# enoche/MMRec

Hardware: NVIDIA H100
Metric: graph-prop edges/sec (+ full-catalog scored-items/sec in extra) @ d=64 (higher is better)
Workload: dtype f32

## Files before the change

include/mmrec_b200.h:

```cpp
#ifndef MMREC_B200_H
#define MMREC_B200_H

#include <stddef.h>
#include <stdint.h>

#ifdef __cplusplus
extern "C" {
#endif

#define MMREC_OK 0
#define MMREC_EINVAL (-1)
#define MMREC_EWORKSPACE (-2)
#define MMREC_ECUDA (-3)
#define MMREC_EUNSUPPORTED (-4)

#define MMREC_ABI_VERSION 3

int mmrec_abi_version(void);
const char* mmrec_last_error(void);
int mmrec_device_check(void);
int64_t mmrec_launch_count(void);

size_t mmrec_csr_from_coo_workspace_bytes(int64_t nnz, int64_t n_rows);
int mmrec_csr_from_coo(int64_t nnz, const int64_t* row, const int64_t* col, const float* val,
// ... 16 lines not shown
                   const int32_t* rowptr, const int32_t* colidx, const float* vals,
                   const int32_t* tasks, int64_t n_tasks, int64_t n_cta_tasks, const int32_t* split_rows,
                   int32_t* counters, float* partial,
                   const float* X, int64_t ldx,
                   float* Y, int64_t ldy,
                   const float* acc_in, float* acc_out, int64_t ldacc, float acc_div,
                   const float* gate_ref, int64_t ldgate,
                   void* stream);

int mmrec_spmm_acc_f32(int64_t n_rows, int64_t n_cols, int d,
                       const int32_t* rowptr, const int32_t* colidx, const float* vals,
                       const int32_t* tasks, int64_t n_tasks, int64_t n_cta_tasks, const int32_t* split_rows,
                       int32_t* counters, float* partial,
                       const float* X, int64_t ldx, float* Y, int64_t ldy,
                       const float* acc_in, float* acc_out, int64_t ldacc, float acc_div, int y_accumulate, void* stream);

int mmrec_spmm_drop_f32(int64_t n_rows, int64_t n_cols, int d,
                        const int32_t* rowptr, const int32_t* colidx, const float* vals,
                        const int32_t* tasks, int64_t n_tasks, int64_t n_cta_tasks, const int32_t* split_rows,
                        int32_t* counters, float* partial,
                        const float* X, int64_t ldx, float* Y, int64_t ldy,
                        const float* acc_in, float* acc_out, int64_t ldacc, float acc_div,
                        const uint32_t* keep_bits, float scale, void* stream);

int mmrec_edge_keep_bits(int64_t nnz, const float* draws, float keep_prob, const int32_t* draw_of, const int32_t* mirror,
                         uint32_t* keep_bits, uint32_t* keep_bits_t, void* stream);

typedef struct {
    int64_t n_rows, n_cols;
    const int32_t* rowptr; const int32_t* colidx; const float* vals;
    const int32_t* tasks; int64_t n_tasks, n_cta_tasks; const int32_t* split_rows; int32_t* counters; float* partial;
    const float* X; int64_t ldx;
    float* Y; int64_t ldy;
    const float* acc_in; float* acc_out; int64_t ldacc; float acc_div;
    const float* post; int64_t ldpost; int64_t post_row0;
    int sync_before;
} mmrec_spmm_step;
int mmrec_spmm_chain_f32(int d, int n_steps, const mmrec_spmm_step* steps, void* stream);

typedef struct {
    mmrec_spmm_step step;
    const float* X_hi; int64_t ldx_hi; int64_t x_split;
    const float* acc_in_hi; int64_t ldacc_in_hi; int64_t acc_in_split;
} mmrec_spmm_step2;
int mmrec_spmm_steps_f32(int d, int n_steps, const mmrec_spmm_step2* steps, int cooperative, void* stream);

int mmrec_project_set_path(int tensor_core);
size_t mmrec_project_workspace_bytes(int64_t n_out, int64_t F, int d);
int mmrec_project_f32(int64_t n_out, const int64_t* idx, const float* table, int64_t n_table, int64_t F,
                      const float* W, const float* bias, int d, int l2_normalize,
                      float* Y, int64_t ldy, void* ws, size_t ws_bytes, void* stream);

int mmrec_debug_mma_rate(int kind, int N, int iters, int distinct, long long* cycles_per_cta, void* stream);

int mmrec_debug_stream_probe(const float* table, int64_t n_rows, int64_t F, int R, int burst_bytes, int ctas_per_sm, float* sink,
                             void* stream);

int mmrec_score_set_path(int path);
size_t mmrec_score_workspace_bytes(int64_t B, int64_t n_items, int d);
int mmrec_score_f32(int64_t B, const int64_t* users, const float* Ue, int64_t ldu,
                    int64_t n_items, const float* Ie, int64_t ldi, int d,
                    float* S, int64_t ldS, void* ws, size_t ws_bytes, void* stream);
int mmrec_mask_f32(int64_t mask_nnz, const int64_t* mask_rows, const int64_t* mask_cols,
                   int64_t B, int64_t n_items, int64_t item_offset, float* S, int64_t ldS, void* stream);
int mmrec_topk_rows_f32(int64_t B, int64_t n_items, const float* S, int64_t ldS, int k,
                        int64_t item_offset, int64_t* out_idx, float* out_val, void* stream);
size_t mmrec_score_topk_workspace_bytes(int64_t B, int64_t n_items, int d, int k);
int mmrec_score_topk_f32(int64_t B, const int64_t* users, const float* Ue, int64_t ldu,
                         int64_t n_items, const float* Ie, int64_t ldi, int d,
                         int64_t mask_nnz, const int64_t* mask_rows, const int64_t* mask_cols,
                         int k, int64_t item_offset, int64_t* out_idx, float* out_val,
                         void* ws, size_t ws_bytes, void* stream);
size_t mmrec_catalog_bytes(int64_t n_items, int d);
int mmrec_catalog_pack_f32(int64_t n_items, const float* Ie, int64_t ldi, int d,
                           void* cat, size_t cat_bytes, void* stream);
int mmrec_score_topk_cat_f32(int64_t B, const int64_t* users, const float* Ue, int64_t ldu,
                             int64_t n_items, const float* Ie, int64_t ldi, int d, const void* cat,
                             int64_t mask_nnz, const int64_t* mask_rows, const int64_t* mask_cols,
                             int k, int64_t item_offset, int64_t* out_idx, float* out_val,
                             void* ws, size_t ws_bytes, void* stream);
int64_t mmrec_debug_fused_fallback_rows(const void* ws, int64_t B, int64_t n_items, int d, int k, int64_t mask_nnz, int with_cat);
int mmrec_debug_cf_scratch(int64_t B, int64_t n_items, int d, int k, int64_t mask_nnz, int with_cat, int64_t* out, int cap);
int mmrec_debug_cf_timing(float* us, int cap);

size_t mmrec_knn_topk_workspace_bytes(int64_t n, int F, int64_t m, int k);
int mmrec_knn_topk_f32(int64_t n, const float* X, int64_t ldx, int F, int64_t m, const int64_t* rows, int k,
                       int64_t* out_idx, float* out_val, void* ws, size_t ws_bytes, void* stream);
int64_t mmrec_debug_knn_fallback_rows(void);
int mmrec_debug_knn_scratch(int64_t n, int F, int64_t m, int k, int64_t* out, int cap);
int mmrec_knn_topk_shrink_f32(int64_t n, const float* X, int64_t ldx, int F, int64_t m, const int64_t* rows, int k,
                              const float* norms, float shrink, int64_t* out_idx, float* out_val, void* ws, size_t ws_bytes,
                              void* stream);

int mmrec_sparse_scores_f32(int64_t B, const int64_t* users, int64_t n_items, const int32_t* r_ptr, const int32_t* r_col,
                            const float* r_val, const int32_t* s_ptr, const int32_t* s_col, const float* s_val, float* out,
                            int64_t ldo, void* stream);
size_t mmrec_sparse_score_topk_workspace_bytes(int64_t B, int64_t n_items, int64_t mask_nnz, int k);
int mmrec_sparse_score_topk_f32(int64_t B, const int64_t* users, int64_t n_items, const int32_t* r_ptr, const int32_t* r_col,
                                const float* r_val, const int32_t* s_ptr, const int32_t* s_col, const float* s_val,
                                int64_t mask_nnz, const int64_t* mask_rows, const int64_t* mask_cols, int k,
                                int64_t* out_idx, float* out_val, void* ws, size_t ws_bytes, void* stream);
int64_t mmrec_debug_sparse_topk_fallback_rows(void);

size_t mmrec_expsum_rows_workspace_bytes(int64_t B, int64_t M, int d);
int mmrec_expsum_rows_f32(int64_t B, const float* Q, int64_t ldq, int64_t M, const float* T, int64_t ldt, int d, float inv_tau,
                          float* ttl, void* ws, size_t ws_bytes, void* stream);
// ... 50 lines not shown
```

mmrec_b200/_lib.py:

```python
from __future__ import annotations

import ctypes as C
import os

_HERE = os.path.dirname(os.path.abspath(__file__))
LIB_PATH = os.path.join(_HERE, "csrc", "libmmrec_b200.so")

_i64, _i32, _f32, _f64, _sz, _p = C.c_int64, C.c_int, C.c_float, C.c_double, C.c_size_t, C.c_void_p

PROTOTYPES = {
    "mmrec_abi_version": (_i32, []),
    "mmrec_last_error": (C.c_char_p, []),
    "mmrec_device_check": (_i32, []),
    "mmrec_launch_count": (_i64, []),
    "mmrec_csr_from_coo_workspace_bytes": (_sz, [_i64, _i64]),
    "mmrec_csr_from_coo": (_i32, [_i64, _p, _p, _p, _i64, _i64, _i32, _p, _p, _p, _p, _p, _sz, _p]),
    "mmrec_spmm_plan_workspace_bytes": (_sz, [_i64, _i64]),
    "mmrec_spmm_plan": (_i32, [_i64, _p, _i32, _i32, _i64, _p, _p, _p, _p, _sz, _p]),
    "mmrec_bipartite_norm_workspace_bytes": (_sz, [_i64, _i64]),
    "mmrec_bipartite_norm_f32": (_i32, [_i64, _p, _p, _i64, _i64, _f32, _p, _p, _sz, _p]),
    "mmrec_spmm_set_lanes": (_i32, [_i32]),
    "mmrec_spmm_f32": (_i32, [_i64, _i64, _i32, _p, _p, _p, _p, _i64, _i64, _p, _p, _p, _p, _i64, _p, _i64, _p, _p, _i64,
                              _f32, _p, _i64, _p]),
    "mmrec_spmm_acc_f32": (_i32, [_i64, _i64, _i32, _p, _p, _p, _p, _i64, _i64, _p, _p, _p, _p, _i64, _p, _i64, _p, _p, _i64,
                                  _f32, _i32, _p]),
    "mmrec_spmm_drop_f32": (_i32, [_i64, _i64, _i32, _p, _p, _p, _p, _i64, _i64, _p, _p, _p, _p, _i64, _p, _i64, _p, _p, _i64,
                                   _f32, _p, _f32, _p]),
    "mmrec_edge_keep_bits": (_i32, [_i64, _p, _f32, _p, _p, _p, _p, _p]),
    "mmrec_spmm_chain_f32": (_i32, [_i32, _i32, _p, _p]),
    "mmrec_spmm_steps_f32": (_i32, [_i32, _i32, _p, _i32, _p]),
    "mmrec_project_set_path": (_i32, [_i32]),
    "mmrec_project_workspace_bytes": (_sz, [_i64, _i64, _i32]),
    "mmrec_project_f32": (_i32, [_i64, _p, _p, _i64, _i64, _p, _p, _i32, _i32, _p, _i64, _p, _sz, _p]),
    "mmrec_debug_mma_rate": (_i32, [_i32, _i32, _i32, _i32, _p, _p]),
    "mmrec_debug_stream_probe": (_i32, [_p, _i64, _i64, _i32, _i32, _i32, _p, _p]),
    "mmrec_score_set_path": (_i32, [_i32]),
    "mmrec_score_workspace_bytes": (_sz, [_i64, _i64, _i32]),
    "mmrec_score_f32": (_i32, [_i64, _p, _p, _i64, _i64, _p, _i64, _i32, _p, _i64, _p, _sz, _p]),
    "mmrec_mask_f32": (_i32, [_i64, _p, _p, _i64, _i64, _i64, _p, _i64, _p]),
    "mmrec_topk_rows_f32": (_i32, [_i64, _i64, _p, _i64, _i32, _i64, _p, _p, _p]),
    "mmrec_score_topk_workspace_bytes": (_sz, [_i64, _i64, _i32, _i32]),
    "mmrec_score_topk_f32": (_i32, [_i64, _p, _p, _i64, _i64, _p, _i64, _i32, _i64, _p, _p, _i32, _i64, _p, _p, _p,
                                    _sz, _p]),
    "mmrec_catalog_bytes": (_sz, [_i64, _i32]),
    "mmrec_catalog_pack_f32": (_i32, [_i64, _p, _i64, _i32, _p, _sz, _p]),
    "mmrec_score_topk_cat_f32": (_i32, [_i64, _p, _p, _i64, _i64, _p, _i64, _i32, _p, _i64, _p, _p, _i32, _i64, _p, _p, _p,
                                        _sz, _p]),
    "mmrec_debug_cf_timing": (_i32, [_p, _i32]),
    "mmrec_debug_fused_fallback_rows": (_i64, [_p, _i64, _i64, _i32, _i32, _i64, _i32]),
    "mmrec_debug_cf_scratch": (_i32, [_i64, _i64, _i32, _i32, _i64, _i32, _p, _i32]),
    "mmrec_knn_topk_workspace_bytes": (_sz, [_i64, _i32, _i64, _i32]),
    "mmrec_knn_topk_f32": (_i32, [_i64, _p, _i64, _i32, _i64, _p, _i32, _p, _p, _p, _sz, _p]),
    "mmrec_debug_knn_fallback_rows": (_i64, []),
    "mmrec_debug_knn_scratch": (_i32, [_i64, _i32, _i64, _i32, _p, _i32]),
    "mmrec_knn_topk_shrink_f32": (_i32, [_i64, _p, _i64, _i32, _i64, _p, _i32, _p, _f32, _p, _p, _p, _sz, _p]),
    "mmrec_sparse_scores_f32": (_i32, [_i64, _p, _i64, _p, _p, _p, _p, _p, _p, _p, _i64, _p]),
    "mmrec_sparse_score_topk_workspace_bytes": (_sz, [_i64, _i64, _i64, _i32]),
    "mmrec_sparse_score_topk_f32": (_i32, [_i64, _p, _i64, _p, _p, _p, _p, _p, _p, _i64, _p, _p, _i32, _p, _p, _p, _sz, _p]),
    "mmrec_debug_sparse_topk_fallback_rows": (_i64, []),
    "mmrec_expsum_rows_workspace_bytes": (_sz, [_i64, _i64, _i32]),
    "mmrec_expsum_rows_f32": (_i32, [_i64, _p, _i64, _i64, _p, _i64, _i32, _f32, _p, _p, _sz, _p]),
    "mmrec_expsum_rows_bwd_f32": (_i32, [_i64, _p, _i64, _i64, _p, _i64, _i32, _f32, _p, _p, _i64, _p, _i64, _p, _sz, _p]),
    "mmrec_topk_merge": (_i32, [_i32, _i64, _i32, _p, _p, _p, _p, _p]),
    "mmrec_topk_merge_peers": (_i32, [_i32, _i64, _i32, _p, _p, _i64, _i64, _i64, _i64, _p, _p, _p, _p, _i32, _p]),
    "mmrec_peer_exchange_f32": (_i32, [_i64, _i32, _i32, _p, _p, _p, _p, _p, _p, _f32, _i32, _p]),
    "mmrec_peer_barrier": (_i32, [_i32, _i32, _p, _p, _p]),
    "mmrec_peer_reduce_push_f32": (_i32, [_i64, _i32, _i32, _p, _p, _p, _p, _f32, _i32, _p]),
    "mmrec_peer_gather_f32": (_i32, [_i64, _i32, _p, _p, _p]),
    "mmrec_topk_metrics_f64": (_i32, [_i64, _i32, _p, _p, _p, _p, _p, _p, _p]),
    "mmrec_peer_sum_f32": (_i32, [_i64, _i32, _p, _p, _p, _f32, _p, _p]),
    "mmrec_index_sum_rows_f32": (_i32, [_i64, _p, _p, _i64, _i32, _i64, _p, _i64, _p]),
    "mmrec_linear_wgrad_workspace_bytes": (_sz, [_i64, _i64, _i32]),
    "mmrec_linear_wgrad_f32": (_i32, [_i64, _p, _p, _i64, _i32, _p, _i64, _i64, _p, _p, _p, _sz, _p]),
    "mmrec_linear_dgrad_f32": (_i32, [_i64, _p, _i64, _i32, _p, _i64, _p, _p]),
    "mmrec_linear_dgrad_adam_f32": (_i32, [_i64, _p, _i64, _i32, _p, _i64, _p, _p, _p, _f64, _f64, _f64, _f64, _f64, _f64, _p]),
    "mmrec_adam_f32": (_i32, [_i32, _p, _f64, _f64, _f64, _f64, _p]),
    "mmrec_gate_rows_f32": (_i32, [_i64, _i32, _p, _p, _p, _p, _p, _p]),
    "mmrec_mgcn_fuse_f32": (_i32, [_i64, _i32, _p, _p, _p, _p, _p, _p, _p, _p, _p, _p, _p, _p, _p]),
}

class SpmmStep(C.Structure):
    _fields_ = [("n_rows", _i64), ("n_cols", _i64), ("rowptr", _p), ("colidx", _p), ("vals", _p),
                ("tasks", _p), ("n_tasks", _i64), ("n_cta_tasks", _i64), ("split_rows", _p), ("counters", _p), ("partial", _p),
                ("X", _p), ("ldx", _i64), ("Y", _p), ("ldy", _i64),
                ("acc_in", _p), ("acc_out", _p), ("ldacc", _i64), ("acc_div", _f32),
                ("post", _p), ("ldpost", _i64), ("post_row0", _i64), ("sync_before", _i32)]

# ... 47 lines not shown
```

mmrec_b200/csrc/project.cu:

```cuda
#include "gemm_simt.cuh"

#include <stdlib.h>
#include <string.h>

using namespace mmrec;

namespace mmrec {
int project_tc(int64_t n_out, const int64_t* idx, const float* table, int64_t F, const float* W, const float* bias, int d,
               int l2_normalize, float* Y, int64_t ldy, void* ws, size_t ws_bytes, cudaStream_t stream);
size_t project_tc_workspace_bytes(int64_t n_out, int64_t F, int d);

static int g_project_path = -1;
static int project_path() {
    if (g_project_path < 0) {
        const char* e = getenv("MMREC_PROJECT_PATH");
        g_project_path = (e && strcmp(e, "simt") == 0) ? 0 : 1;
    }
    return g_project_path;
}

__global__ void project_generic_kernel(int64_t n_out, const int64_t* __restrict__ idx, const float* __restrict__ table,
                                       int64_t F, const float* __restrict__ W, const float* __restrict__ bias, int d,
                                       int l2, float* __restrict__ Y, int64_t ldy) {
    extern __shared__ float sh[];
    __shared__ float red[32];
    const int64_t n = blockIdx.x;
    const float* x = table + (idx ? idx[n] : n) * F;
    float ss = 0.f;
    for (int c = threadIdx.x; c < d; c += blockDim.x) {
        const float* w = W + (int64_t)c * F;
        float acc = 0.f;
        for (int64_t k = 0; k < F; ++k) acc = fmaf(x[k], w[k], acc);
        if (bias) acc += bias[c];
        sh[c] = acc;
        ss += acc * acc;
    }
    if (l2) {
        ss = warp_sum(ss);
        if ((threadIdx.x & 31) == 0) red[threadIdx.x >> 5] = ss;
        __syncthreads();
        if (threadIdx.x < 32) {
            float v = threadIdx.x < (blockDim.x >> 5) ? red[threadIdx.x] : 0.f;
            v = warp_sum(v);
            if (threadIdx.x == 0) red[0] = v;
        }
        __syncthreads();
    } else {
        __syncthreads();
    }
    const float inv = l2 ? 1.0f / fmaxf(sqrtf(red[0]), 1e-12f) : 1.0f;
    for (int c = threadIdx.x; c < d; c += blockDim.x) Y[n * ldy + c] = l2 ? sh[c] * inv : sh[c];
}
}

extern "C" int mmrec_project_set_path(int tensor_core) { g_project_path = tensor_core ? 1 : 0; return MMREC_OK; }

extern "C" size_t mmrec_project_workspace_bytes(int64_t n_out, int64_t F, int d) {
    return project_tc_workspace_bytes(n_out, F, d) + 256;
}

extern "C" int mmrec_project_f32(int64_t n_out, const int64_t* idx, const float* table, int64_t n_table, int64_t F,
                                 const float* W, const float* bias, int d, int l2_normalize, float* Y, int64_t ldy,
                                 void* ws, size_t ws_bytes, void* stream_) {
    cudaStream_t stream = (cudaStream_t)stream_;
    MMREC_CHECK_ARG(n_out >= 0 && n_table >= 0 && F >= 1 && d >= 1, "project: bad sizes");
    if (n_out == 0) return MMREC_OK;
    MMREC_CHECK_ARG(table && W && Y && ldy >= d, "project: null pointer or ldy < d");
    if (project_path() == 1 && ws) {
        int r = project_tc(n_out, idx, table, F, W, bias, d, l2_normalize, Y, ldy, ws, ws_bytes, stream);
        if (r != 0) return r < 0 ? r : MMREC_OK;
    }
    GemmNT p;
    p.A = table; p.lda = F; p.a_idx = idx; p.M = n_out;
    p.B = W; p.ldb = F; p.N = d; p.K = F; p.bias = bias; p.C = Y; p.ldc = ldy; p.l2_normalize = l2_normalize;
    if (d <= 32) return launch_gemm_nt<64, 32, 4, 2>(p, stream);
    if (d <= 64) return launch_gemm_nt<32, 64, 2, 4>(p, stream);
    if (d <= 128) return launch_gemm_nt<32, 128, 2, 8>(p, stream);
    if (d <= 256) return launch_gemm_nt<32, 256, 2, 16>(p, stream);
    project_generic_kernel<<<(unsigned)n_out, 128, (size_t)d * sizeof(float), stream>>>(n_out, idx, table, F, W, bias, d,
                                                                                   l2_normalize, Y, ldy);
    MMREC_LAUNCH_CHECK();
    return MMREC_OK;
}

namespace mmrec {
__global__ void __launch_bounds__(256) stream_probe_kernel(const float4* __restrict__ table, int64_t n_rows, int64_t row_f4, int R, int burst_f4,
                                                           float* __restrict__ sink) {
    const int tiles = (int)((n_rows + R - 1) / R);
    float acc = 0.f;
    for (int tile = blockIdx.x; tile < tiles; tile += gridDim.x) {
        for (int64_t o = 0; o < row_f4; o += burst_f4) {
            float4 v[16];
#pragma unroll
            for (int i = 0; i < 16; ++i) {
                const int e = i * 256 + threadIdx.x;
                const int r = e / burst_f4, c = e - r * burst_f4;
                const int64_t row = (int64_t)tile * R + r;
                v[i] = (r < R && row < n_rows && o + c < row_f4) ? __ldg(table + row * row_f4 + o + c) : make_float4(0.f, 0.f, 0.f, 0.f);
            }
#pragma unroll
            for (int i = 0; i < 16; ++i) acc += v[i].x + v[i].y + v[i].z + v[i].w;
        }
    }
    if (acc == 123.456f) *sink = acc;
}
}

extern "C" int mmrec_debug_stream_probe(const float* table, int64_t n_rows, int64_t F, int R, int burst_bytes, int ctas_per_sm, float* sink,
                                        void* stream_) {
    MMREC_CHECK_ARG(table && sink && (F & 3) == 0 && R >= 1 && burst_bytes >= 16 && (int64_t)R * burst_bytes == 65536 && ctas_per_sm >= 1,
                    "stream_probe: need R * burst_bytes == 65536");
    mmrec::stream_probe_kernel<<<(unsigned)(mmrec::sm_count() * ctas_per_sm), 256, 0, (cudaStream_t)stream_>>>(
        (const float4*)table, n_rows, F / 4, R, burst_bytes / 16, sink);
    MMREC_LAUNCH_CHECK();
    return MMREC_OK;
}
```

mmrec_b200/csrc/project_tc.cu:

```cuda
#include "tc_common.cuh"

namespace mmrec {

using namespace tc;

constexpr int PJ_M = 128;
constexpr int PJ_KC = 32;
constexpr int PJ_LBO_A = 2064;
constexpr int PJ_A_BYTES = (PJ_KC / 4) * PJ_LBO_A;
constexpr int PJ_CONV = 256;
constexpr int PJ_THREADS = PJ_CONV + 32;
template <int N> constexpr int pj_depth() { return N == 64 ? 3 : (N == 128 ? 2 : 1); }

struct ProjParams {
    const float* table; int64_t F; const int64_t* idx; int64_t n_out;
    const float *Whi, *Wlo;
    int N, n_chunks, chunks_per_split, n_splits, stages, vec_ok, n_tiles;
    float* partial;
    int64_t rows_padded;
};

struct PjSmem {
    uint32_t a0, b0, bars, total, stage_bytes, b_bytes;
};
__host__ __device__ inline PjSmem pj_smem(int N, int stages) {
    PjSmem L;
    L.b_bytes = (uint32_t)N * PJ_KC * 4;
    L.stage_bytes = 2 * PJ_A_BYTES + 2 * L.b_bytes;
    L.a0 = 0;
    L.b0 = 2 * PJ_A_BYTES;
    L.bars = stages * L.stage_bytes;
    L.total = L.bars + 32 * 8;
    return L;
}

template <int N, bool FAST>
__global__ void __launch_bounds__(PJ_THREADS, 1) project_tc_kernel(const ProjParams p) {
    constexpr int PJ_DEPTH = pj_depth<N>();
    extern __shared__ __align__(1024) uint8_t smem[];
    const PjSmem L = pj_smem(N, p.stages);
    const uint32_t sbase = smem_u32(smem);
    const uint32_t bar = sbase + L.bars;
    const int warp = threadIdx.x >> 5, lane = threadIdx.x & 31;
    if (threadIdx.x == 0) {
        for (int s = 0; s < 8; ++s) { mbar_init(bar + s * 8, PJ_CONV); mbar_init(bar + (8 + s) * 8, 1); mbar_init(bar + (16 + s) * 8, PJ_CONV / 32); }
        mbar_fence_init();
    }
    __syncthreads();

    const int tile = blockIdx.x / p.n_splits, sp = blockIdx.x % p.n_splits;
    const int c0 = sp * p.chunks_per_split;
    const int c1 = min(p.n_chunks, c0 + p.chunks_per_split);
// ... 67 lines not shown
    uint32_t par = 1;
    int done = 0;
    auto fill = [&](int cbase, float4 (&ring)[PJ_DEPTH][4]) {
#pragma unroll
        for (int q = 0; q < PJ_DEPTH; ++q) load_chunk(cbase + q, ring[q]);
    };
    auto drain = [&](int cbase, float4 (&ring)[PJ_DEPTH][4]) {
#pragma unroll
        for (int q = 0; q < PJ_DEPTH; ++q) {
            if (cbase + q < n_my) {
                mbar_wait(bar + (16 + s) * 8, par);
                uint8_t* st = smem + s * L.stage_bytes;
#pragma unroll
                for (int i = 0; i < 4; ++i) {
                    const int r = (t >> 3) + 32 * i;
                    const uint32_t off = kb * PJ_LBO_A + (r >> 3) * 128 + (r & 7) * 16;
                    float4 h, l;
                    split_tf32_trunc(ring[q][i].x, h.x, l.x); split_tf32_trunc(ring[q][i].y, h.y, l.y);
                    split_tf32_trunc(ring[q][i].z, h.z, l.z); split_tf32_trunc(ring[q][i].w, h.w, l.w);
                    *reinterpret_cast<float4*>(st + L.a0 + off) = h;
                    *reinterpret_cast<float4*>(st + L.a0 + PJ_A_BYTES + off) = l;
                }
                fence_proxy_async();
                mbar_arrive(bar + s * 8);
                mbar_wait(bar + s * 8, par ^ 1);
                mbar_wait(bar + (8 + s) * 8, par ^ 1);
                const uint64_t st_off = (uint64_t)(s * L.stage_bytes) >> 4;
                uint64_t a_hi = a_hi0 + st_off, a_lo = a_lo0 + st_off, b_hi = b_hi0 + st_off, b_lo = b_lo0 + st_off;
                wgmma_fence();
#pragma unroll
                for (int j = 0; j < PJ_KC / 8; ++j) {
                    wgmma_tf32<N>(acc, a_hi, b_hi, first);
                    first = 1;
                    wgmma_tf32<N>(acc, a_lo, b_hi, 1);
                    wgmma_tf32<N>(acc, a_hi, b_lo, 1);
                    a_hi += ka; a_lo += ka; b_hi += kbs; b_lo += kbs;
                }
                wgmma_commit();
                if (done++ > 0) {
                    wgmma_wait<1>();
                    warp_arrive(bar + (16 + prev) * 8);
                }
                prev = s;
                if (++s == p.stages) { s = 0; par ^= 1; }
            }
        }
    };
    fill(0, ringA);
    for (int cb = 0; cb < n_my; cb += 2 * PJ_DEPTH) {
        fill(cb + PJ_DEPTH, ringB);
        drain(cb, ringA);
        fill(cb + 2 * PJ_DEPTH, ringA);
        drain(cb + PJ_DEPTH, ringB);
    }
    wgmma_wait<0>();
    wgmma_fence_regs(acc);
    const int w = (t >> 5) & 3;
    const int64_t row0 = (int64_t)tile * PJ_M + g * 64 + w * 16 + (lane >> 2);
#pragma unroll
    for (int h = 0; h < 2; ++h) {
        float* dst = p.partial + ((int64_t)sp * p.rows_padded + row0 + 8 * h) * N + 2 * (lane & 3);
#pragma unroll
        for (int j = 0; j < N / 8; ++j)
            *reinterpret_cast<float2*>(dst + 8 * j) = make_float2(acc[4 * j + 2 * h], acc[4 * j + 2 * h + 1]);
    }
}

__global__ void __launch_bounds__(256) project_reduce_kernel(int64_t n_out, int d, int N, int n_splits, int64_t rows_padded,
                                                             const float* __restrict__ partial, const float* __restrict__ bias,
                                                             int l2, float* __restrict__ Y, int64_t ldy) {
    const int lane = threadIdx.x & 31;
    const int64_t row = (int64_t)blockIdx.x * 8 + (threadIdx.x >> 5);
    if (row >= n_out) return;
    float acc[8];
    float ss = 0.f;
#pragma unroll
    for (int i = 0; i < 8; ++i) {
        const int c = lane + 32 * i;
        float a = 0.f;
        if (c < d) {
            for (int s = 0; s < n_splits; ++s) a += partial[((int64_t)s * rows_padded + row) * N + c];
            if (bias) a += __ldg(bias + c);
            ss += a * a;
        }
        acc[i] = a;
    }
    float inv = 1.f;
    if (l2) { ss = warp_sum(ss); inv = 1.0f / fmaxf(sqrtf(ss), 1e-12f); }
#pragma unroll
    for (int i = 0; i < 8; ++i) {
        const int c = lane + 32 * i;
        if (c < d) Y[row * ldy + c] = l2 ? acc[i] * inv : acc[i];
    }
}

struct PjPlan {
    int N, KP, n_chunks, n_splits, chunks_per_split, stages;
    int64_t n_tiles, rows_padded;
    size_t off_whi, off_wlo, off_partial, total;
};

static bool pj_plan(int64_t n_out, int64_t F, int d, PjPlan& P) {
    if (d > 256 || n_out <= 0 || F < 1) return false;
    P.N = d <= 64 ? 64 : (d <= 128 ? 128 : 256);
    P.KP = (int)((F + PJ_KC - 1) / PJ_KC * PJ_KC);
    P.n_chunks = P.KP / PJ_KC;
    P.n_tiles = (n_out + PJ_M - 1) / PJ_M;
    P.rows_padded = P.n_tiles * PJ_M;
    const int sms = sm_count();
    int splits = (int)(sms / P.n_tiles);
    if (splits < 1) splits = 1;
    if (splits > P.n_chunks / 4) splits = P.n_chunks / 4 > 0 ? P.n_chunks / 4 : 1;
    if (splits > 32) splits = 32;
    P.chunks_per_split = (P.n_chunks + splits - 1) / splits;
    P.n_splits = (P.n_chunks + P.chunks_per_split - 1) / P.chunks_per_split;
    const uint32_t stage = 2 * PJ_A_BYTES + 2 * (uint32_t)P.N * PJ_KC * 4;
    P.stages = (int)((220 * 1024) / stage);
    if (P.stages > 8) P.stages = 8;
    if (P.stages < 2) return false;
    size_t off = 0;
    auto take = [&](size_t bytes) { size_t o = off; off += align_up(bytes, 1024); return o; };
    P.off_whi = take((size_t)P.N * P.KP * 4);
    P.off_wlo = take((size_t)P.N * P.KP * 4);
    P.off_partial = take((size_t)P.n_splits * P.rows_padded * P.N * 4);
    P.total = off + 1024;
    return true;
}

size_t project_tc_workspace_bytes(int64_t n_out, int64_t F, int d) {
    PjPlan P;
    return pj_plan(n_out, F, d, P) ? P.total : 0;
}

template <int R>
static int pack_weights(const float* W, int64_t F, int d, int KP, float* hi, float* lo, cudaStream_t stream) {
    const int64_t total = (int64_t)R * (KP / 4);
    pack_split_kernel<R><<<(unsigned)((total + 255) / 256), 256, 0, stream>>>(d, nullptr, W, F, (int)F, KP, hi, lo, 1);
    MMREC_LAUNCH_CHECK();
    return MMREC_OK;
}

int project_tc(int64_t n_out, const int64_t* idx, const float* table, int64_t F, const float* W, const float* bias, int d,
               int l2_normalize, float* Y, int64_t ldy, void* ws, size_t ws_bytes, cudaStream_t stream) {
    PjPlan P;
    if (!ws || !pj_plan(n_out, F, d, P) || ws_bytes < P.total || F >= (1ll << 31)) return 0;
    char* base = (char*)(((uintptr_t)ws + 1023) & ~(uintptr_t)1023);
    float *Whi = (float*)(base + P.off_whi), *Wlo = (float*)(base + P.off_wlo), *partial = (float*)(base + P.off_partial);
    int rc = P.N == 64 ? pack_weights<64>(W, F, d, P.KP, Whi, Wlo, stream)
                       : (P.N == 128 ? pack_weights<128>(W, F, d, P.KP, Whi, Wlo, stream) : pack_weights<256>(W, F, d, P.KP, Whi, Wlo, stream));
    if (rc) return rc;
    ProjParams p;
    p.table = table; p.F = F; p.idx = idx; p.n_out = n_out; p.Whi = Whi; p.Wlo = Wlo; p.N = P.N; p.n_chunks = P.n_chunks;
    p.chunks_per_split = P.chunks_per_split; p.n_splits = P.n_splits; p.stages = P.stages;
    p.n_tiles = (int)P.n_tiles;
    p.vec_ok = ((F & 3) == 0) && ((((uintptr_t)table) & 15) == 0);
    p.partial = partial; p.rows_padded = P.rows_padded;
    const PjSmem L = pj_smem(P.N, P.stages);
    rc = set_smem_once<project_tc_kernel<64, true>, project_tc_kernel<64, false>, project_tc_kernel<128, true>,
                       project_tc_kernel<128, false>, project_tc_kernel<256, true>, project_tc_kernel<256, false>>(227 * 1024);
    if (rc) return rc;
    const bool fast = p.vec_ok && (F % PJ_KC) == 0;
    const unsigned grid = (unsigned)(P.n_tiles * P.n_splits);
    if (P.N == 64) {
        if (fast) project_tc_kernel<64, true><<<grid, PJ_THREADS, L.total, stream>>>(p);
        else project_tc_kernel<64, false><<<grid, PJ_THREADS, L.total, stream>>>(p);
    } else if (P.N == 128) {
        if (fast) project_tc_kernel<128, true><<<grid, PJ_THREADS, L.total, stream>>>(p);
        else project_tc_kernel<128, false><<<grid, PJ_THREADS, L.total, stream>>>(p);
    } else {
        if (fast) project_tc_kernel<256, true><<<grid, PJ_THREADS, L.total, stream>>>(p);
        else project_tc_kernel<256, false><<<grid, PJ_THREADS, L.total, stream>>>(p);
    }
    MMREC_LAUNCH_CHECK();
    project_reduce_kernel<<<(unsigned)((n_out + 7) / 8), 256, 0, stream>>>(n_out, d, P.N, P.n_splits, P.rows_padded, partial, bias,
                                                                         l2_normalize, Y, ldy);
    MMREC_LAUNCH_CHECK();
    return 1;
}

}
```

mmrec_b200/csrc/spmm.cu:

```cuda
#include <cooperative_groups.h>

#include "common.cuh"

namespace mmrec {

struct SpmmParams {
    int64_t n_rows, n_cols;
    const int32_t* rowptr; const int32_t* colidx; const float* vals;
    const int4* tasks; int64_t n_tasks, n_heavy; const int4* split_rows; int32_t* counters; float* partial;
    const float* X; int64_t ldx;
    float* Y; int64_t ldy;
    const float* acc_in; float* acc_out; int64_t ldacc; float acc_div;
    const float* gate_ref; int64_t ldgate;
    int y_acc;
    const float* post; int64_t post_row0; uint32_t spost;
    int d;
    uint32_t sx, sy, sacc, sgate;
    const float* X_hi; const float* acc_in_hi;
    int x_split, acc_split;
    uint32_t sx_hi, sacc_hi;
};


__device__ __forceinline__ const float4* row_f4(const float* base, uint32_t stride, int r, int f4) {
// ... 235 lines not shown
                }
            }
            bool do_epi = g == 0 && sid < 0;
            if (sid >= 0) do_epi = spmm_split_finish<D, T, TWO>(p, g == 0, row, tk.y, sid, l, acc, accin);
            spmm_epilogue<D, T>(p, do_epi, row, l, acc, accin);
        }
        __syncthreads();
    }

    const int64_t W = (int64_t)gridDim.x * (blockDim.x >> 5);
    const int64_t w = (int64_t)blockIdx.x * (blockDim.x >> 5) + warp;
    const int64_t n_light = n_work - n_heavy;
    auto slot_of = [&](int64_t it) -> int64_t { return it * W + ((it & 1) ? (W - 1 - w) : w); };
    auto fetch = [&](int64_t slot) -> int4 {
        const int64_t t = slot * C::GPW + g;
        if (t >= n_light) return make_int4(-1, 0, 0, -1);
        if (p.tasks) return __ldg(p.tasks + n_heavy + t);
        return make_int4((int)t, __ldg(p.rowptr + t), __ldg(p.rowptr + t + 1), -1);
    };
    const int64_t n_slots = (n_light + C::GPW - 1) / C::GPW;
    const int64_t n_iter = (n_slots + W - 1) / W;
    int4 nxt = fetch(slot_of(0));
    for (int64_t it = 0; it < n_iter; ++it) {
        const int row = nxt.x, b = nxt.y, sid = nxt.w;
        const int len = nxt.z - nxt.y;
        const bool valid = row >= 0;
        nxt = fetch(slot_of(it + 1));
        const int maxlen = __reduce_max_sync(0xffffffffu, valid ? len : 0);
        float4 accin[C::V];
#pragma unroll
        for (int v = 0; v < C::V; ++v) accin[v] = make_float4(0.f, 0.f, 0.f, 0.f);
        if (valid && p.acc_in && sid < 0) {
#pragma unroll
            for (int v = 0; v < C::V; ++v)
                accin[v] = acc_in_f4<TWO>(p, row, v * T + l);
        }
        float4 acc[C::V];
#pragma unroll
        for (int v = 0; v < C::V; ++v) acc[v] = make_float4(0.f, 0.f, 0.f, 0.f);
        spmm_gather<D, T, TWO, DROP>(p, b, valid ? len : 0, maxlen, l, acc, dk);
        bool do_epi = valid && sid < 0;
        const bool split = valid && sid >= 0;
        if (__any_sync(0xffffffffu, split)) {
            if (spmm_split_finish<D, T, TWO>(p, split, row, b, sid, l, acc, accin)) do_epi = true;
        }
        spmm_epilogue<D, T>(p, do_epi, row, l, acc, accin);
    }
}

template <int D, int T>
__global__ void __launch_bounds__(256) spmm_vec_kernel(const SpmmParams p) {
    __shared__ __align__(16) float red[(256 / T) * D];
    spmm_vec_body<D, T, false>(p, red);
}

template <int D, int T>
__global__ void __launch_bounds__(256) spmm_drop_kernel(const SpmmParams p, const uint32_t* __restrict__ keep, float scale) {
    __shared__ __align__(16) float red[(256 / T) * D];
    spmm_vec_body<D, T, false, true>(p, red, DropKeep{keep, scale});
}

__global__ void __launch_bounds__(256) edge_keep_bits_kernel(int64_t nnz, const float* __restrict__ draws, float keep_prob,
                                                             const int32_t* __restrict__ draw_of, const int32_t* __restrict__ mirror,
                                                             uint32_t* __restrict__ keep, uint32_t* __restrict__ keep_t) {
    const int64_t n_words = (nnz + 31) >> 5;
    const int lane = threadIdx.x & 31;
    const int64_t w0 = ((int64_t)blockIdx.x * blockDim.x + threadIdx.x) >> 5;
    const int64_t n_warps = ((int64_t)gridDim.x * blockDim.x) >> 5;
    auto kept = [&](int64_t e) { return floorf(__fadd_rn(keep_prob, __ldg(draws + __ldg(draw_of + e)))) != 0.f; };
    for (int64_t w = w0; w < n_words; w += n_warps) {
        const int64_t e = (w << 5) + lane;
        const bool in = e < nnz;
        const uint32_t word = __ballot_sync(0xffffffffu, in && kept(e));
        const uint32_t word_t = keep_t ? __ballot_sync(0xffffffffu, in && kept(__ldg(mirror + e))) : 0u;
        if (lane == 0) {
            keep[w] = word;
            if (keep_t) keep_t[w] = word_t;
        }
    }
}

constexpr int SPMM_CHAIN_MAX = 8;
struct SpmmChain { SpmmParams step[SPMM_CHAIN_MAX]; int n; unsigned sync_mask; };

template <int D, int T, bool COOP>
__global__ void __launch_bounds__(256, 3) spmm_chain_kernel(const SpmmChain c) {
    __shared__ __align__(16) float red[(256 / T) * D];
    for (int i = 0; i < c.n; ++i) {
        if (COOP && ((c.sync_mask >> i) & 1u)) { __threadfence(); cooperative_groups::this_grid().sync(); }
        spmm_vec_body<D, T, true>(c.step[i], red);
    }
}

__global__ void __launch_bounds__(256) spmm_generic_kernel(const SpmmParams p) {
    const int lane = threadIdx.x & 31;
    const int64_t warp0 = (int64_t)blockIdx.x * (blockDim.x >> 5) + (threadIdx.x >> 5);
    const int64_t nwarps = (int64_t)gridDim.x * (blockDim.x >> 5);
    for (int64_t row = warp0; row < p.n_rows; row += nwarps) {
        const int b = p.rowptr[row], e = p.rowptr[row + 1];
        float dot = 0.f, ny = 0.f, nr = 0.f;
        if (p.gate_ref) {
            for (int k0 = 0; k0 < p.d; k0 += 32) {
                const int k = k0 + lane;
                float acc = 0.f;
                if (k < p.d)
                    for (int j = b; j < e; ++j) acc = fmaf(p.vals[j], p.X[(int64_t)p.colidx[j] * p.ldx + k], acc);
// ... 305 lines not shown
```

mmrec_b200/csrc/tc_common.cuh:

```cuda
#pragma once
#include <cuda_fp16.h>

#include "common.cuh"
#include "wgmma.cuh"

namespace mmrec {
namespace tc {

__device__ __forceinline__ uint32_t smem_u32(const void* p) { return (uint32_t)__cvta_generic_to_shared(p); }

__device__ __forceinline__ void mbar_init(uint32_t bar, uint32_t count) {
    asm volatile("mbarrier.init.shared::cta.b64 [%0], %1;" ::"r"(bar), "r"(count) : "memory");
}
__device__ __forceinline__ void mbar_fence_init() { asm volatile("fence.mbarrier_init.release.cluster;" ::: "memory"); }
__device__ __forceinline__ void mbar_arrive(uint32_t bar) {
    asm volatile("mbarrier.arrive.shared::cta.b64 _, [%0];" ::"r"(bar) : "memory");
}
__device__ __forceinline__ void mbar_expect_tx(uint32_t bar, uint32_t bytes) {
    asm volatile("mbarrier.arrive.expect_tx.shared::cta.b64 _, [%0], %1;" ::"r"(bar), "r"(bytes) : "memory");
}
__device__ __forceinline__ bool mbar_try_wait(uint32_t bar, uint32_t parity) {
    uint32_t ok;
    asm volatile(
        "{\n\t.reg .pred p;\n\t"
        "mbarrier.try_wait.parity.shared::cta.b64 p, [%1], %2;\n\t"
        "selp.u32 %0, 1, 0, p;\n\t}"
        : "=r"(ok) : "r"(bar), "r"(parity) : "memory");
    return ok != 0;
}
__device__ __forceinline__ uint64_t global_ns() {
    uint64_t t;
    asm volatile("mov.u64 %0, %%globaltimer;" : "=l"(t));
    return t;
}
__device__ __forceinline__ void mbar_wait(uint32_t bar, uint32_t parity) {
    uint32_t spins = 0;
    uint64_t t0 = 0;
    while (!mbar_try_wait(bar, parity)) {
        if (++spins == 4096u) t0 = global_ns();
        if (spins > 4096u && (spins & 1023u) == 0 && global_ns() - t0 > 2000000000ull) __trap();
    }
}

__device__ __forceinline__ void bulk_g2s(uint32_t dst_smem, const void* src, uint32_t bytes, uint32_t bar) {
    asm volatile("cp.async.bulk.shared::cluster.global.mbarrier::complete_tx::bytes [%0], [%1], %2, [%3];"
                 ::"r"(dst_smem), "l"(src), "r"(bytes), "r"(bar) : "memory");
}

__device__ __forceinline__ void wgmma_fence() { asm volatile("wgmma.fence.sync.aligned;" ::: "memory"); }
__device__ __forceinline__ void wgmma_commit() { asm volatile("wgmma.commit_group.sync.aligned;" ::: "memory"); }
template <int N>
__device__ __forceinline__ void wgmma_wait() { asm volatile("wgmma.wait_group.sync.aligned %0;" ::"n"(N) : "memory"); }
template <int R>
__device__ __forceinline__ void wgmma_fence_regs(float (&d)[R]) {
#pragma unroll
    for (int i = 0; i < R; ++i) asm volatile("" : "+f"(d[i])::"memory");
}
__device__ __forceinline__ void fence_proxy_async() { asm volatile("fence.proxy.async.shared::cta;" ::: "memory"); }
__device__ __forceinline__ void warp_arrive(uint32_t bar) {
    __syncwarp();
    if ((threadIdx.x & 31) == 0) mbar_arrive(bar);
}

__device__ __forceinline__ uint64_t smem_desc(uint32_t smem_addr, uint32_t lbo_bytes, uint32_t sbo_bytes) {
    uint64_t d = 0;
    d |= (uint64_t)((smem_addr & 0x3FFFFu) >> 4);
    d |= (uint64_t)((lbo_bytes >> 4) & 0x3FFFu) << 16;
    d |= (uint64_t)((sbo_bytes >> 4) & 0x3FFFu) << 32;
    return d;
}

__device__ __forceinline__ void split_tf32(float x, float& hi, float& lo) {
    uint32_t h, l;
    asm("cvt.rna.tf32.f32 %0, %1;" : "=r"(h) : "f"(x));
    hi = __uint_as_float(h);
    asm("cvt.rna.tf32.f32 %0, %1;" : "=r"(l) : "f"(x - hi));
    lo = __uint_as_float(l);
}

__device__ __forceinline__ void split_tf32_trunc(float x, float& hi, float& lo) {
    hi = __uint_as_float(__float_as_uint(x) & 0xffffe000u);
    lo = x - hi;
}

}

__device__ __forceinline__ float fp16_scale_for(uint32_t m_bits) {
    const uint32_t e = (m_bits >> 23) & 0xffu;
    if (e == 0u || e == 255u || e < 14u) return 1.0f;
    return __uint_as_float((268u - e) << 23);
}

__global__ void absmax_norm_kernel(int64_t n, const float* __restrict__ X, int64_t ldx, int F, float* __restrict__ rnorm,
                                   uint32_t* __restrict__ amax, uint32_t* __restrict__ nmax);

__device__ __forceinline__ void store_fp16x8(uint4* __restrict__ out, int64_t tile, int kblks, int kb, int rr, const float (&x)[8], float sc) {
    uint32_t w[4];
#pragma unroll
    for (int e = 0; e < 4; ++e) {
        const __half2 h = __floats2half2_rn(x[2 * e] * sc, x[2 * e + 1] * sc);
        w[e] = *reinterpret_cast<const uint32_t*>(&h);
    }
    out[((tile * kblks + kb) * 16 + rr / 8) * 8 + (rr % 8)] = make_uint4(w[0], w[1], w[2], w[3]);
}

template <int GPT, class Dst>
__device__ __forceinline__ void group_max_store(const float (&acc)[64], int e2, int q, int n_valid, int64_t row, int64_t n_rows, Dst dst) {
    auto val = [&](int j, int e) { return 8 * j + 2 * q + e < n_valid ? acc[4 * j + 2 * e2 + e] : -INFINITY; };
    float gm[GPT];
#pragma unroll
    for (int g = 0; g < GPT; ++g) {
        float m = -INFINITY;
#pragma unroll
        for (int j = g * (16 / GPT); j < (g + 1) * (16 / GPT); ++j) m = fmaxf(m, fmaxf(val(j, 0), val(j, 1)));
        m = fmaxf(m, __shfl_xor_sync(0xffffffffu, m, 1));
        gm[g] = fmaxf(m, __shfl_xor_sync(0xffffffffu, m, 2));
    }
    if (row < n_rows) {
        float* d = dst();
#pragma unroll
        for (int g = 0; g < GPT; ++g)
            if ((g & 3) == q) d[g] = gm[g];
// ... 47 lines not shown
```

Measured before the change: 13.76 billion.

## Add TMA-fed projection kernel, tf32 trunc probe, and occupancy bound for spmm d=64

Adds a new projection path that loads the feature table with a TMA tensor map into 128B-swizzled shared memory and splits it into hi/lo parts in place, so the raw value is used directly as the hi operand. It also adds a debug probe for truncated-tf32 wgmma behaviour. Separately, it specialises the d=64, T=16 spmm vector kernel with a minimum of 4 blocks per SM in its launch bounds, capping registers to raise occupancy for graph propagation. The measured metric is spmm edges/sec, so the launch-bounds change is the part that matters for it. It risks register spills.

```diff
diff --git a/include/mmrec_b200.h b/include/mmrec_b200.h
--- a/include/mmrec_b200.h
+++ b/include/mmrec_b200.h
@@ -92,6 +92,8 @@
                       float* Y, int64_t ldy, void* ws, size_t ws_bytes, void* stream);
 
 int mmrec_debug_mma_rate(int kind, int N, int iters, int distinct, long long* cycles_per_cta, void* stream);
+
+int mmrec_debug_tf32_trunc(const float* A, const float* B, float* out, void* stream);
 
 int mmrec_debug_stream_probe(const float* table, int64_t n_rows, int64_t F, int R, int burst_bytes, int ctas_per_sm, float* sink,
                              void* stream);
diff --git a/mmrec_b200/_lib.py b/mmrec_b200/_lib.py
--- a/mmrec_b200/_lib.py
+++ b/mmrec_b200/_lib.py
@@ -33,6 +33,7 @@
     "mmrec_project_workspace_bytes": (_sz, [_i64, _i64, _i32]),
     "mmrec_project_f32": (_i32, [_i64, _p, _p, _i64, _i64, _p, _p, _i32, _i32, _p, _i64, _p, _sz, _p]),
     "mmrec_debug_mma_rate": (_i32, [_i32, _i32, _i32, _i32, _p, _p]),
+    "mmrec_debug_tf32_trunc": (_i32, [_p, _p, _p, _p]),
     "mmrec_debug_stream_probe": (_i32, [_p, _i64, _i64, _i32, _i32, _i32, _p, _p]),
     "mmrec_score_set_path": (_i32, [_i32]),
     "mmrec_score_workspace_bytes": (_sz, [_i64, _i64, _i32]),
diff --git a/mmrec_b200/csrc/project.cu b/mmrec_b200/csrc/project.cu
--- a/mmrec_b200/csrc/project.cu
+++ b/mmrec_b200/csrc/project.cu
@@ -7,7 +7,7 @@
 
 namespace mmrec {
 int project_tc(int64_t n_out, const int64_t* idx, const float* table, int64_t F, const float* W, const float* bias, int d,
-               int l2_normalize, float* Y, int64_t ldy, void* ws, size_t ws_bytes, cudaStream_t stream);
+               int l2_normalize, float* Y, int64_t ldy, void* ws, size_t ws_bytes, cudaStream_t stream, bool register_feed);
 size_t project_tc_workspace_bytes(int64_t n_out, int64_t F, int d);
 
 static int g_project_path = -1;
@@ -53,7 +53,7 @@
 }
 }
 
-extern "C" int mmrec_project_set_path(int tensor_core) { g_project_path = tensor_core ? 1 : 0; return MMREC_OK; }
+extern "C" int mmrec_project_set_path(int tensor_core) { g_project_path = tensor_core == 2 ? 2 : (tensor_core ? 1 : 0); return MMREC_OK; }
 
 extern "C" size_t mmrec_project_workspace_bytes(int64_t n_out, int64_t F, int d) {
     return project_tc_workspace_bytes(n_out, F, d) + 256;
@@ -66,8 +66,8 @@
     MMREC_CHECK_ARG(n_out >= 0 && n_table >= 0 && F >= 1 && d >= 1, "project: bad sizes");
     if (n_out == 0) return MMREC_OK;
     MMREC_CHECK_ARG(table && W && Y && ldy >= d, "project: null pointer or ldy < d");
-    if (project_path() == 1 && ws) {
-        int r = project_tc(n_out, idx, table, F, W, bias, d, l2_normalize, Y, ldy, ws, ws_bytes, stream);
+    if (project_path() >= 1 && ws) {
+        int r = project_tc(n_out, idx, table, F, W, bias, d, l2_normalize, Y, ldy, ws, ws_bytes, stream, project_path() == 2);
         if (r != 0) return r < 0 ? r : MMREC_OK;
     }
     GemmNT p;
diff --git a/mmrec_b200/csrc/project_tc.cu b/mmrec_b200/csrc/project_tc.cu
--- a/mmrec_b200/csrc/project_tc.cu
+++ b/mmrec_b200/csrc/project_tc.cu
@@ -1,3 +1,5 @@
+#include <cudaTypedefs.h>
+
 #include "tc_common.cuh"
 
 namespace mmrec {
@@ -171,6 +173,108 @@
         drain(cb, ringA);
         fill(cb + 2 * PJ_DEPTH, ringA);
         drain(cb + PJ_DEPTH, ringB);
+    }
+    wgmma_wait<0>();
+    wgmma_fence_regs(acc);
+    const int w = (t >> 5) & 3;
+    const int64_t row0 = (int64_t)tile * PJ_M + g * 64 + w * 16 + (lane >> 2);
+#pragma unroll
+    for (int h = 0; h < 2; ++h) {
+        float* dst = p.partial + ((int64_t)sp * p.rows_padded + row0 + 8 * h) * N + 2 * (lane & 3);
+#pragma unroll
+        for (int j = 0; j < N / 8; ++j)
+            *reinterpret_cast<float2*>(dst + 8 * j) = make_float2(acc[4 * j + 2 * h], acc[4 * j + 2 * h + 1]);
+    }
+}
+
+constexpr int PJT_TILE_BYTES = PJ_M * PJ_KC * 4;
+__host__ __device__ inline uint32_t pjt_stage_bytes(int N) { return 2 * PJT_TILE_BYTES + 2 * (uint32_t)N * PJ_KC * 4; }
+__host__ __device__ inline uint32_t pjt_bars(int N, int stages) { return 1024 + stages * pjt_stage_bytes(N); }
+
+template <int N>
+__global__ void __launch_bounds__(PJ_THREADS, 1) project_tma_kernel(const __grid_constant__ CUtensorMap tmap, const ProjParams p) {
+    extern __shared__ __align__(1024) uint8_t smem_raw[];
+    const uint32_t sraw = smem_u32(smem_raw);
+    const uint32_t sbase = (sraw + 1023u) & ~1023u;
+    uint8_t* smem = smem_raw + (sbase - sraw);
+    const uint32_t stage_bytes = pjt_stage_bytes(N), b_bytes = (uint32_t)N * PJ_KC * 4;
+    const uint32_t bar = sraw + pjt_bars(N, p.stages);
+    const int warp = threadIdx.x >> 5, lane = threadIdx.x & 31;
+    if (threadIdx.x == 0) {
+        for (int s = 0; s < 8; ++s) { mbar_init(bar + s * 8, 1); mbar_init(bar + (8 + s) * 8, PJ_CONV / 32); }
+        mbar_fence_init();
+    }
+    __syncthreads();
+
+    const int tile = blockIdx.x / p.n_splits, sp = blockIdx.x % p.n_splits;
+    const int c0 = sp * p.chunks_per_split;
+    const int c1 = min(p.n_chunks, c0 + p.chunks_per_split);
+    const int n_my = c1 - c0;
+    constexpr int PJ_DEPTH = pj_depth<N>();
+    const int rot = n_my > 0 ? ((int)(((int64_t)tile * n_my) / p.n_tiles) / PJ_DEPTH * PJ_DEPTH) % n_my : 0;
+
+    if (warp == PJ_CONV / 32) {
+        if (lane == 0) {
+            int s = 0;
+            uint32_t par = 1;
+            for (int c = 0; c < n_my; ++c) {
+                mbar_wait(bar + (8 + s) * 8, par);
+                const uint32_t full = bar + s * 8, st = sbase + s * stage_bytes;
+                mbar_expect_tx(full, PJT_TILE_BYTES + 2 * b_bytes);
+                const int kc = c0 + (c + rot) % n_my;
+                tma_load_2d(st, &tmap, kc * PJ_KC, tile * PJ_M, full);
+                const int64_t off = (int64_t)kc * (b_bytes / 4);
+                bulk_g2s(st + 2 * PJT_TILE_BYTES, p.Whi + off, b_bytes, full);
+                bulk_g2s(st + 2 * PJT_TILE_BYTES + b_bytes, p.Wlo + off, b_bytes, full);
+                if (++s == p.stages) { s = 0; par ^= 1; }
+            }
+        }
+        return;
+    }
+    const int t = threadIdx.x;
+    const int g = t >> 7;
+    const uint32_t LBO_B = (uint32_t)(N / 8) * 128;
+    const uint64_t a_raw0 = smem_desc_sw128(sbase + g * (PJT_TILE_BYTES / 2)), a_lo0 = smem_desc_sw128(sbase + PJT_TILE_BYTES + g * (PJT_TILE_BYTES / 2));
+    const uint64_t b_hi0 = smem_desc(sbase + 2 * PJT_TILE_BYTES, LBO_B, 128), b_lo0 = smem_desc(sbase + 2 * PJT_TILE_BYTES + b_bytes, LBO_B, 128);
+    const uint64_t ka = (8 * 4) >> 4, kbs = (2 * LBO_B) >> 4;
+    float acc[N / 2];
+#pragma unroll
+    for (int i = 0; i < N / 2; ++i) acc[i] = 0.f;
+    uint32_t first = 0;
+    int s = 0, prev = 0;
+    uint32_t par = 1;
+    for (int c = 0; c < n_my; ++c) {
+        mbar_wait(bar + s * 8, par ^ 1);
+        uint8_t* half = smem + s * stage_bytes + g * (PJT_TILE_BYTES / 2);
+#pragma unroll
+        for (int i = 0; i < 4; ++i) {
+            const uint32_t off = ((t & 127) + 128 * i) * 16;
+            const float4 x = *reinterpret_cast<const float4*>(half + off);
+            float4 h, l;
+            split_tf32_trunc(x.x, h.x, l.x); split_tf32_trunc(x.y, h.y, l.y);
+            split_tf32_trunc(x.z, h.z, l.z); split_tf32_trunc(x.w, h.w, l.w);
+            *reinterpret_cast<float4*>(half + PJT_TILE_BYTES + off) = l;
+        }
+        fence_proxy_async();
+        named_bar_sync(1 + g, 128);
+        const uint64_t st_off = (uint64_t)(s * stage_bytes) >> 4;
+        uint64_t a_raw = a_raw0 + st_off, a_lo = a_lo0 + st_off, b_hi = b_hi0 + st_off, b_lo = b_lo0 + st_off;
+        wgmma_fence();
+#pragma unroll
+        for (int j = 0; j < PJ_KC / 8; ++j) {
+            wgmma_tf32<N>(acc, a_raw, b_hi, first);
+            first = 1;
+            wgmma_tf32<N>(acc, a_lo, b_hi, 1);
+            wgmma_tf32<N>(acc, a_raw, b_lo, 1);
+            a_raw += ka; a_lo += ka; b_hi += kbs; b_lo += kbs;
+        }
+        wgmma_commit();
+        if (c > 0) {
+            wgmma_wait<1>();
+            warp_arrive(bar + (8 + prev) * 8);
+        }
+        prev = s;
+        if (++s == p.stages) { s = 0; par ^= 1; }
     }
     wgmma_wait<0>();
     wgmma_fence_regs(acc);
@@ -259,8 +363,63 @@
     return MMREC_OK;
 }
 
+static PFN_cuTensorMapEncodeTiled_v12000 tensor_map_encoder() {
+    static const PFN_cuTensorMapEncodeTiled_v12000 fn = [] {
+        void* f = nullptr;
+        cudaDriverEntryPointQueryResult q = cudaDriverEntryPointSymbolNotFound;
+        if (cudaGetDriverEntryPointByVersion("cuTensorMapEncodeTiled", &f, 12000, cudaEnableDefault, &q) != cudaSuccess ||
+            q != cudaDriverEntryPointSuccess)
+            f = nullptr;
+        return (PFN_cuTensorMapEncodeTiled_v12000)f;
+    }();
+    return fn;
+}
+
+static int pjt_stages(int N) {
+    const int s = (int)((220 * 1024 - 1024) / pjt_stage_bytes(N));
+    return s < 2 ? 0 : (s > 8 ? 8 : s);
+}
+
+template <int N>
+static int launch_project_tma(const ProjParams& p, unsigned grid, cudaStream_t stream) {
+    const PFN_cuTensorMapEncodeTiled_v12000 encode = tensor_map_encoder();
+    MMREC_CHECK_ARG(encode, "project: the driver has no cuTensorMapEncodeTiled");
+    CUtensorMap map;
+    const cuuint64_t dims[2] = {(cuuint64_t)p.F, (cuuint64_t)p.n_out};
+    const cuuint64_t strides[1] = {(cuuint64_t)p.F * 4};
+    const cuuint32_t box[2] = {PJ_KC, PJ_M}, estr[2] = {1, 1};
+    const CUresult r = encode(&map, CU_TENSOR_MAP_DATA_TYPE_FLOAT32, 2, (void*)p.table, dims, strides, box, estr,
+                              CU_TENSOR_MAP_INTERLEAVE_NONE, CU_TENSOR_MAP_SWIZZLE_128B, CU_TENSOR_MAP_L2_PROMOTION_L2_256B,
+                              CU_TENSOR_MAP_FLOAT_OOB_FILL_NONE);
+    MMREC_CHECK_ARG(r == CUDA_SUCCESS, "project: cuTensorMapEncodeTiled failed (%d)", (int)r);
+    int rc = set_smem_once<project_tma_kernel<N>>(227 * 1024);
+    if (rc) return rc;
+    project_tma_kernel<N><<<grid, PJ_THREADS, pjt_bars(N, p.stages) + 16 * 8, stream>>>(map, p);
+    MMREC_LAUNCH_CHECK();
+    return MMREC_OK;
+}
+
+static int launch_project_regs(const ProjParams& p, const PjPlan& P, bool fast, unsigned grid, cudaStream_t stream) {
+    const PjSmem L = pj_smem(P.N, P.stages);
+    int rc = set_smem_once<project_tc_kernel<64, true>, project_tc_kernel<64, false>, project_tc_kernel<128, true>,
+                           project_tc_kernel<128, false>, project_tc_kernel<256, true>, project_tc_kernel<256, false>>(227 * 1024);
+    if (rc) return rc;
+    if (P.N == 64) {
+        if (fast) project_tc_kernel<64, true><<<grid, PJ_THREADS, L.total, stream>>>(p);
+        else project_tc_kernel<64, false><<<grid, PJ_THREADS, L.total, stream>>>(p);
+    } else if (P.N == 128) {
+        if (fast) project_tc_kernel<128, true><<<grid, PJ_THREADS, L.total, stream>>>(p);
+        else project_tc_kernel<128, false><<<grid, PJ_THREADS, L.total, stream>>>(p);
+    } else {
+        if (fast) project_tc_kernel<256, true><<<grid, PJ_THREADS, L.total, stream>>>(p);
+        else project_tc_kernel<256, false><<<grid, PJ_THREADS, L.total, stream>>>(p);
+    }
+    MMREC_LAUNCH_CHECK();
+    return MMREC_OK;
+}
+
 int project_tc(int64_t n_out, const int64_t* idx, const float* table, int64_t F, const float* W, const float* bias, int d,
-               int l2_normalize, float* Y, int64_t ldy, void* ws, size_t ws_bytes, cudaStream_t stream) {
+               int l2_normalize, float* Y, int64_t ldy, void* ws, size_t ws_bytes, cudaStream_t stream, bool register_feed) {
     PjPlan P;
     if (!ws || !pj_plan(n_out, F, d, P) || ws_bytes < P.total || F >= (1ll << 31)) return 0;
     char* base = (char*)(((uintptr_t)ws + 1023) & ~(uintptr_t)1023);
@@ -274,27 +433,61 @@
     p.n_tiles = (int)P.n_tiles;
     p.vec_ok = ((F & 3) == 0) && ((((uintptr_t)table) & 15) == 0);
     p.partial = partial; p.rows_padded = P.rows_padded;
-    const PjSmem L = pj_smem(P.N, P.stages);
-    rc = set_smem_once<project_tc_kernel<64, true>, project_tc_kernel<64, false>, project_tc_kernel<128, true>,
-                       project_tc_kernel<128, false>, project_tc_kernel<256, true>, project_tc_kernel<256, false>>(227 * 1024);
-    if (rc) return rc;
     const bool fast = p.vec_ok && (F % PJ_KC) == 0;
     const unsigned grid = (unsigned)(P.n_tiles * P.n_splits);
-    if (P.N == 64) {
-        if (fast) project_tc_kernel<64, true><<<grid, PJ_THREADS, L.total, stream>>>(p);
-        else project_tc_kernel<64, false><<<grid, PJ_THREADS, L.total, stream>>>(p);
-    } else if (P.N == 128) {
-        if (fast) project_tc_kernel<128, true><<<grid, PJ_THREADS, L.total, stream>>>(p);
-        else project_tc_kernel<128, false><<<grid, PJ_THREADS, L.total, stream>>>(p);
+    if (fast && !idx && !register_feed && pjt_stages(P.N) > 0 && n_out < (1ll << 31) - PJ_M) {
+        p.stages = pjt_stages(P.N);
+        rc = P.N == 64 ? launch_project_tma<64>(p, grid, stream)
+                       : (P.N == 128 ? launch_project_tma<128>(p, grid, stream) : launch_project_tma<256>(p, grid, stream));
     } else {
-        if (fast) project_tc_kernel<256, true><<<grid, PJ_THREADS, L.total, stream>>>(p);
-        else project_tc_kernel<256, false><<<grid, PJ_THREADS, L.total, stream>>>(p);
-    }
-    MMREC_LAUNCH_CHECK();
+        rc = launch_project_regs(p, P, fast, grid, stream);
+    }
+    if (rc) return rc;
     project_reduce_kernel<<<(unsigned)((n_out + 7) / 8), 256, 0, stream>>>(n_out, d, P.N, P.n_splits, P.rows_padded, partial, bias,
                                                                          l2_normalize, Y, ldy);
     MMREC_LAUNCH_CHECK();
     return 1;
 }
 
-}
+__global__ void __launch_bounds__(128) tf32_trunc_probe_kernel(const float* __restrict__ A, const float* __restrict__ B, float* __restrict__ out) {
+    __shared__ __align__(1024) float sa[2][64 * 8], sb[64 * 8];
+    const int t = threadIdx.x;
+    for (int e = t; e < 64 * 8; e += 128) {
+        const int r = e / 8, k = e % 8;
+        const int o = (k / 4) * 256 + (r / 8) * 32 + (r % 8) * 4 + k % 4;
+        float h, l;
+        split_tf32_trunc(A[e], h, l);
+        sa[0][o] = A[e];
+        sa[1][o] = h;
+        sb[o] = B[e];
+    }
+    fence_proxy_async();
+    __syncthreads();
+    const uint64_t b = smem_desc(smem_u32(sb), 1024, 128);
+#pragma unroll
+    for (int v = 0; v < 2; ++v) {
+        float acc[32];
+#pragma unroll
+        for (int i = 0; i < 32; ++i) acc[i] = 0.f;
+        wgmma_fence();
+        wgmma_tf32<64>(acc, smem_desc(smem_u32(sa[v]), 1024, 128), b, 0);
+        wgmma_commit();
+        wgmma_wait<0>();
+        wgmma_fence_regs(acc);
+        const int w = t >> 5, lane = t & 31;
+#pragma unroll
+        for (int j = 0; j < 8; ++j)
+#pragma unroll
+            for (int e = 0; e < 4; ++e)
+                out[(v * 64 + 16 * w + (lane >> 2) + 8 * (e >> 1)) * 64 + 8 * j + 2 * (lane & 3) + (e & 1)] = acc[4 * j + e];
+    }
+}
+
+}
+
+extern "C" int mmrec_debug_tf32_trunc(const float* A, const float* B, float* out, void* stream_) {
+    MMREC_CHECK_ARG(A && B && out, "debug_tf32_trunc: null pointer");
+    mmrec::tf32_trunc_probe_kernel<<<1, 128, 0, (cudaStream_t)stream_>>>(A, B, out);
+    MMREC_LAUNCH_CHECK();
+    return MMREC_OK;
+}
diff --git a/mmrec_b200/csrc/spmm.cu b/mmrec_b200/csrc/spmm.cu
--- a/mmrec_b200/csrc/spmm.cu
+++ b/mmrec_b200/csrc/spmm.cu
@@ -311,6 +311,11 @@
 __global__ void __launch_bounds__(256) spmm_vec_kernel(const SpmmParams p) {
     __shared__ __align__(16) float red[(256 / T) * D];
     spmm_vec_body<D, T, false>(p, red);
+}
+template <>
+__global__ void __launch_bounds__(256, 4) spmm_vec_kernel<64, 16>(const SpmmParams p) {
+    __shared__ __align__(16) float red[(256 / 16) * 64];
+    spmm_vec_body<64, 16, false>(p, red);
 }
 
 template <int D, int T>
diff --git a/mmrec_b200/csrc/tc_common.cuh b/mmrec_b200/csrc/tc_common.cuh
--- a/mmrec_b200/csrc/tc_common.cuh
+++ b/mmrec_b200/csrc/tc_common.cuh
@@ -68,6 +68,22 @@
     d |= (uint64_t)((lbo_bytes >> 4) & 0x3FFFu) << 16;
     d |= (uint64_t)((sbo_bytes >> 4) & 0x3FFFu) << 32;
     return d;
+}
+__device__ __forceinline__ uint64_t smem_desc_sw128(uint32_t smem_addr) {
+    uint64_t d = 0;
+    d |= (uint64_t)((smem_addr & 0x3FFFFu) >> 4);
+    d |= (uint64_t)1u << 16;
+    d |= (uint64_t)(1024u >> 4) << 32;
+    d |= (uint64_t)1u << 62;
+    return d;
+}
+
+__device__ __forceinline__ void tma_load_2d(uint32_t dst_smem, const void* tmap, int x, int y, uint32_t bar) {
+    asm volatile("cp.async.bulk.tensor.2d.shared::cluster.global.tile.mbarrier::complete_tx::bytes [%0], [%1, {%2, %3}], [%4];"
+                 ::"r"(dst_smem), "l"(tmap), "r"(x), "r"(y), "r"(bar) : "memory");
+}
+__device__ __forceinline__ void named_bar_sync(int id, int threads) {
+    asm volatile("bar.sync %0, %1;" ::"r"(id), "r"(threads) : "memory");
 }
 
 __device__ __forceinline__ void split_tf32(float x, float& hi, float& lo) {
```

Result: faster. 15.11 billion (median of 6 runs) (+9.8%).
